# arkworks-rs/sponge

Measured on AMD Instinct MI355X. Metric: Poseidon permutations/sec (BLS12-381 Fr, t=3), higher is better.
Workload: dtype u32

## Files before the change

### sponge_amd/csrc/pmx_field.hpp

```cpp
#pragma once
#include <cstdint>
#include <type_traits>

#if defined(__HIPCC__)
#include <hip/hip_runtime.h>
#define PMX_FN __host__ __device__ __forceinline__
#else
#define PMX_FN inline
#endif

#if defined(PMX_HOSTCHECK) && !defined(__HIPCC__)
#define PMX_TRACK(tag, x, f) ::pmx::hostcheck_track(tag, x, f)
#else
#define PMX_TRACK(tag, x, f) ((void)0)
#endif

namespace pmx {

constexpr int kW = 29;
constexpr int kN = 9;
constexpr uint32_t kMask = (1u << kW) - 1;
constexpr int kFeStride = 12;

#if defined(__HIP_DEVICE_COMPILE__)
// ... 33 lines not shown
    uint32_t p[kN];
    uint32_t pinv;
    uint32_t unit;
    const uint32_t *io;
};
constexpr int kIoP32 = 0, kIoToInt = 8, kIoToAbi = 8 + kN, kIoFromU64 = 28, kIoWords = 40;

#if defined(PMX_HOSTCHECK) && !defined(__HIPCC__)
void hostcheck_track(int tag, const Fe &x, const FieldRt &f);
void hostcheck_below_2_256(const Fe &x);
#endif

PMX_FN Fe fe_const(const uint32_t *ptr) {
    Fe r;
#pragma unroll
    for (int i = 0; i < kN; ++i) r.l[i] = ptr[i];
    return r;
}

PMX_FN Fe fe_zero() {
    Fe z;
#pragma unroll
    for (int i = 0; i < kN; ++i) z.l[i] = 0;
    return z;
}

PMX_FN uint32_t mont_step(uint64_t &acc, const FieldRt &f) {
    const uint32_t m = ((uint32_t)acc * f.pinv) & kMask;
    acc += (uint64_t)m * f.p[0];
    acc >>= kW;
    return m;
}

PMX_FN Fe fe_add_lazy(const Fe &a, const Fe &b) {
    Fe r;
#pragma unroll
    for (int i = 0; i < kN; ++i) r.l[i] = a.l[i] + b.l[i];
    return r;
}

PMX_FN Fe fe_normalize(const Fe &a) {
    Fe r;
    uint32_t carry = 0;
#pragma unroll
    for (int i = 0; i < kN - 1; ++i) {
        const uint32_t v = a.l[i] + carry;
        r.l[i] = v & kMask;
        carry = v >> kW;
    }
    r.l[kN - 1] = a.l[kN - 1] + carry;
    return r;
}

template <int T, bool ADD>
PMX_FN Fe mont_dot_impl(const Fe *a, const Fe *b, const Fe &s, const FieldRt &f) {
    constexpr int G = (T + 2) / 3;
    uint32_t m[kN];
    Fe out;
    uint64_t acc[G];
#pragma unroll
    for (int g = 0; g < G; ++g) acc[g] = 0;
#pragma unroll
    for (int k = 0; k < 2 * kN - 1; ++k) {
        const int lo_i = k < kN ? 0 : k - (kN - 1);
        const int hi_i = k < kN ? k : kN - 1;
#pragma unroll
        for (int t = 0; t < T; ++t) {
#pragma unroll
            for (int i = lo_i; i <= hi_i; ++i) acc[t / 3] += (uint64_t)a[t].l[i] * b[t].l[k - i];
        }
#pragma unroll
        for (int j = lo_i; j <= hi_i; ++j) {
            if (j < k || k >= kN) acc[0] += (uint64_t)m[j] * f.p[k - j];
        }
        if constexpr (G == 1) {
            if (k < kN) {
                m[k] = mont_step(acc[0], f);
            } else {
                if constexpr (ADD) acc[0] += (uint64_t)s.l[k - kN] * f.unit;
                out.l[k - kN] = (uint32_t)acc[0] & kMask;
                acc[0] >>= kW;
            }
        } else {
            uint32_t low = (uint32_t)acc[0] & kMask;
            if constexpr (ADD) {
                if (k >= kN) low += s.l[k - kN];
            }
            uint64_t carry = acc[0] >> kW;
#pragma unroll
            for (int g = 1; g < G; ++g) {
                low += (uint32_t)acc[g] & kMask;
                carry += acc[g] >> kW;
                acc[g] = 0;
            }
            if (k < kN) {
                m[k] = (low * f.pinv) & kMask;
                const uint64_t v = (uint64_t)m[k] * f.p[0] + low;
                acc[0] = carry + (v >> kW);
            } else {
                out.l[k - kN] = low & kMask;
                acc[0] = carry + (low >> kW);
            }
        }
    }
    out.l[kN - 1] = (uint32_t)acc[0];
    if constexpr (ADD) out.l[kN - 1] += s.l[kN - 1];
    return out;
}

template <int T>
PMX_FN Fe mont_dot(const Fe *a, const Fe *b, const FieldRt &f) { return mont_dot_impl<T, false>(a, b, a[0], f); }
template <int T>
PMX_FN Fe mont_dot_add(const Fe *a, const Fe *b, const Fe &s, const FieldRt &f) { return mont_dot_impl<T, true>(a, b, s, f); }

PMX_FN Fe mont_mul(const Fe &a, const Fe &b, const FieldRt &f) { return mont_dot<1>(&a, &b, f); }

PMX_FN Fe mont_mul_add(const Fe &a, const Fe &b, const Fe &s, const FieldRt &f) {
    uint32_t m[kN];
    Fe out;
    uint64_t acc = 0;
#pragma unroll
    for (int k = 0; k < 2 * kN - 1; ++k) {
        const int lo_i = k < kN ? 0 : k - (kN - 1);
        const int hi_i = k < kN ? k : kN - 1;
#pragma unroll
        for (int i = lo_i; i <= hi_i; ++i) acc += (uint64_t)a.l[i] * b.l[k - i];
#pragma unroll
        for (int j = lo_i; j <= hi_i; ++j) {
            if (j < k || k >= kN) acc += (uint64_t)m[j] * f.p[k - j];
        }
        if (k < kN) {
            m[k] = mont_step(acc, f);
        } else {
            acc += (uint64_t)s.l[k - kN] * f.unit;
            out.l[k - kN] = (uint32_t)acc & kMask;
            acc >>= kW;
        }
    }
    out.l[kN - 1] = (uint32_t)acc + s.l[kN - 1];
    return out;
}

PMX_FN Fe mont_sqr(const Fe &a, const FieldRt &f) {
    uint32_t d[kN];
#pragma unroll
    for (int i = 0; i < kN; ++i) d[i] = a.l[i] << 1;
    uint32_t m[kN];
    Fe out;
    uint64_t acc = 0;
#pragma unroll
    for (int k = 0; k < 2 * kN - 1; ++k) {
#pragma unroll
        for (int i = 0; i < kN; ++i) {
            const int j = k - i;
            if (j > i && j < kN) acc += (uint64_t)a.l[i] * d[j];
        }
        if ((k & 1) == 0) acc += (uint64_t)a.l[k / 2] * a.l[k / 2];
        if (k < kN) {
#pragma unroll
            for (int j = 0; j < k; ++j) acc += (uint64_t)m[j] * f.p[k - j];
            m[k] = mont_step(acc, f);
        } else {
#pragma unroll
            for (int j = k - (kN - 1); j < kN; ++j) acc += (uint64_t)m[j] * f.p[k - j];
            out.l[k - kN] = (uint32_t)acc & kMask;
            acc >>= kW;
        }
    }
    out.l[kN - 1] = (uint32_t)acc;
    return out;
}

enum { kP1In = 0, kP1Sq = 1, kP1Out = 2 };
PMX_FN constexpr bool field_unit_low_limb(const uint32_t (&p)[kN]) { return p[0] == 1u; }

PMX_FN uint32_t mont_step_p1(uint64_t &acc) {
    const uint32_t n = ~(uint32_t)acc & kMask;
    acc >>= kW;
    return n;
}

PMX_FN Fe mont_mul_p1(const Fe &a, const Fe &b, const FieldRt &f) {
    uint32_t m[kN];
    Fe out;
    uint64_t acc = 0;
#pragma unroll
    for (int k = 0; k < 2 * kN - 1; ++k) {
        const int lo_i = k < kN ? 0 : k - (kN - 1);
        const int hi_i = k < kN ? k : kN - 1;
#pragma unroll
        for (int i = lo_i; i <= hi_i; ++i) acc += (uint64_t)a.l[i] * b.l[k - i];
#pragma unroll
        for (int j = lo_i; j <= hi_i; ++j) {
            if (j < k || k >= kN) acc += (uint64_t)m[j] * f.p[k - j];
        }
        if (k < kN) {
            if (k == kN - 1) acc += (uint64_t)1 << kW;
            m[k] = mont_step_p1(acc);
            if (k == 0) m[0] += 1;
        } else {
            out.l[k - kN] = (uint32_t)acc & kMask;
            acc >>= kW;
        }
    }
    out.l[kN - 1] = (uint32_t)acc;
    return out;
}

template <int MODE>
PMX_FN Fe mont_sqr_p1(const Fe &a, const FieldRt &f) {
    uint32_t d[kN];
#pragma unroll
    for (int i = 0; i < kN; ++i) d[i] = a.l[i] << 1;
    uint32_t m[kN];
    Fe out;
    uint64_t acc = MODE == kP1Sq ? ~(uint64_t)0 : (uint64_t)0;
#pragma unroll
    for (int k = 0; k < 2 * kN - 1; ++k) {
#pragma unroll
        for (int i = 0; i < kN; ++i) {
            const int j = k - i;
            if (j > i && j < kN) acc += (uint64_t)a.l[i] * d[j];
        }
        if ((k & 1) == 0) acc += (uint64_t)a.l[k / 2] * a.l[k / 2];
        if (k < kN) {
#pragma unroll
            for (int j = 0; j < k; ++j) acc += (uint64_t)m[j] * f.p[k - j];
            if (MODE == kP1Out && k == kN - 1) acc += (uint64_t)1 << kW;
            m[k] = mont_step_p1(acc);
            if (MODE != kP1Sq && k == 0) m[0] += 1;
        } else {
#pragma unroll
            for (int j = k - (kN - 1); j < kN; ++j) acc += (uint64_t)m[j] * f.p[k - j];
            out.l[k - kN] = (uint32_t)acc & kMask;
            acc >>= kW;
        }
    }
    out.l[kN - 1] = (uint32_t)acc;
    if (MODE != kP1Out) out.l[0] += 1;
    return out;
}

constexpr int kTabSteps = 2;
constexpr int kTabChunk = 3;
constexpr int kTabChunkWords = 32;
constexpr int kTabOneWords = (kN / kTabChunk) * kTabChunkWords;
PMX_FN constexpr int tab_row_words(int n) { return n == 1 ? kTabOneWords : kN * ((n + kTabChunk - 1) / kTabChunk) * kTabChunkWords; }
template <int N>
PMX_FN constexpr int tab_index(int i, int k, int j) {
    return N == 1 ? (k / kTabChunk) * kTabChunkWords + (k % kTabChunk) * kN + j
                  : (k * ((N + kTabChunk - 1) / kTabChunk) + i / kTabChunk) * kTabChunkWords + (i % kTabChunk) * kN + j;
}

PMX_FN void tab_col_end(int k, uint64_t &acc, uint32_t (&m)[kTabSteps], Fe &out, const Fe &s, const FieldRt &f) {
#pragma unroll
    for (int q = 0; q < kTabSteps; ++q) {
        if (q < k && k - q < kN) acc += (uint64_t)m[q] * f.p[k - q];
    }
    if (k < kTabSteps) {
// ... 38 lines not shown
            s[l] = out;
            acc = 0;
        }
        PMX_STREAM_FENCE(acc);
    });
}

struct Cols {
    uint64_t c[2 * kN];
};

PMX_FN void cols_zero(Cols &t) {
#pragma unroll
    for (int k = 0; k < 2 * kN; ++k) t.c[k] = 0;
}

PMX_FN void cols_mul_acc(Cols &t, const Fe &a, const Fe &b) {
#pragma unroll
    for (int i = 0; i < kN; ++i) {
#pragma unroll
        for (int j = 0; j < kN; ++j) t.c[i + j] += (uint64_t)a.l[i] * b.l[j];
    }
}

PMX_FN void cols_compress(Cols &t) {
#pragma unroll
    for (int k = 0; k < 2 * kN - 1; ++k) {
        t.c[k + 1] += t.c[k] >> kW;
        t.c[k] &= kMask;
    }
}

template <bool ADD = false>
PMX_FN Fe cols_redc(Cols &t, const FieldRt &f, const Fe *s = nullptr) {
#pragma unroll
    for (int k = 0; k < kN; ++k) {
        const uint32_t m = ((uint32_t)t.c[k] * f.pinv) & kMask;
#pragma unroll
        for (int j = 0; j < kN; ++j) t.c[k + j] += (uint64_t)m * f.p[j];
        t.c[k + 1] += t.c[k] >> kW;
    }
    Fe out;
#pragma unroll
    for (int k = kN; k < 2 * kN - 1; ++k) {
        if constexpr (ADD) t.c[k] += (uint64_t)s->l[k - kN] * f.unit;
        out.l[k - kN] = (uint32_t)t.c[k] & kMask;
        t.c[k + 1] += t.c[k] >> kW;
    }
    out.l[kN - 1] = (uint32_t)t.c[2 * kN - 1];
    if constexpr (ADD) out.l[kN - 1] += s->l[kN - 1];
    return out;
}

template <int ALPHA, bool P1 = false>
PMX_FN Fe fe_sbox(const Fe &x, uint64_t alpha, const Fe &one, const FieldRt &f) {
    if constexpr (P1 && ALPHA == 5) {
        const Fe x2 = mont_sqr_p1<kP1In>(x, f);
        const Fe x4 = mont_sqr_p1<kP1Sq>(x2, f);
        return mont_mul_p1(x4, x, f);
    } else if constexpr (P1 && ALPHA == 17) {
        Fe y = mont_sqr_p1<kP1In>(x, f);
        y = mont_sqr_p1<kP1Sq>(y, f);
        y = mont_sqr_p1<kP1Sq>(y, f);
        y = mont_sqr_p1<kP1Sq>(y, f);
        return mont_mul_p1(y, x, f);
    } else if constexpr (P1) {
        if (alpha == 0) return one;
        if (alpha == 1) return mont_mul_p1(x, one, f);
        const int top = 63 - __builtin_clzll(alpha);
        Fe acc = mont_sqr_p1<kP1Out>(x, f);
        if ((alpha >> (top - 1)) & 1) acc = mont_mul_p1(acc, x, f);
        for (int bit = top - 2; bit >= 0; --bit) {
            acc = mont_sqr_p1<kP1Out>(acc, f);
            if ((alpha >> bit) & 1) acc = mont_mul_p1(acc, x, f);
        }
        return acc;
    } else if constexpr (ALPHA == 5) {
        const Fe x2 = mont_sqr(x, f);
        const Fe x4 = mont_sqr(x2, f);
        return mont_mul(x4, x, f);
    } else if constexpr (ALPHA == 17) {
        Fe y = mont_sqr(x, f);
        y = mont_sqr(y, f);
        y = mont_sqr(y, f);
        y = mont_sqr(y, f);
        return mont_mul(y, x, f);
    } else {
        if (alpha == 0) return one;
        if (alpha == 1) return mont_mul(x, one, f);
        const int top = 63 - __builtin_clzll(alpha);
        Fe acc = mont_sqr(x, f);
        if ((alpha >> (top - 1)) & 1) acc = mont_mul(acc, x, f);
        for (int bit = top - 2; bit >= 0; --bit) {
            acc = mont_sqr(acc, f);
            if ((alpha >> bit) & 1) acc = mont_mul(acc, x, f);
        }
        return acc;
    }
}

PMX_FN Fe limbs_32_to_29(const Abi &x) {
    Fe r;
#pragma unroll
    for (int i = 0; i < kN; ++i) {
        const int bit = kW * i, wi = bit / 32, sh = bit % 32;
        uint64_t pair = x.w[wi];
        if (wi + 1 < 8) pair |= (uint64_t)x.w[wi + 1] << 32;
        r.l[i] = (uint32_t)(pair >> sh) & kMask;
    }
    return r;
}

PMX_FN Abi limbs_29_to_32(const Fe &x) {
    Abi r;
#pragma unroll
    for (int k = 0; k < 8; ++k) {
        const int bit = 32 * k, li = bit / kW, sh = bit % kW;
        uint64_t v = (uint64_t)x.l[li] >> sh;
        if (li + 1 < kN) v |= (uint64_t)x.l[li + 1] << (kW - sh);
        if (li + 2 < kN && 2 * kW - sh < 32) v |= (uint64_t)x.l[li + 2] << (2 * kW - sh);
        r.w[k] = (uint32_t)v;
    }
    return r;
}

PMX_FN Fe fe_from_abi(const Abi &x, const FieldRt &f) { return mont_mul(limbs_32_to_29(x), fe_const(f.io + kIoToInt), f); }

PMX_FN Abi fe_to_abi(const Fe &x, const FieldRt &f) {
    const Abi t = limbs_29_to_32(mont_mul(x, fe_const(f.io + kIoToAbi), f));
    uint32_t d[8];
    uint32_t borrow = 0;
#pragma unroll
    for (int i = 0; i < 8; ++i) {
        const uint64_t v = (uint64_t)t.w[i] - f.io[kIoP32 + i] - borrow;
        d[i] = (uint32_t)v;
        borrow = (uint32_t)(v >> 32) & 1u;
    }
    Abi r;
#pragma unroll
// ... 126 lines not shown
```

### sponge_amd/csrc/pmx_mfma.hpp

```cpp
#pragma once

#include "pmx_field.hpp"

namespace pmx {

#define PMX_MFMA_MIN_T 3
#define PMX_MFMA_MAX_T 9
constexpr int kMfmaElemBytes = 32;
constexpr int kMfmaShift = 24;
PMX_FN constexpr int mfma_k_steps(int t) { return (t * kMfmaElemBytes + 31) / 32; }
PMX_FN constexpr int mfma_row_words(int t) { return mfma_k_steps(t) * 64 * 4; }
PMX_FN constexpr int mfma_layer_words(int t) { return t * mfma_row_words(t) + t * 16; }
PMX_FN constexpr int mfma_layer_words_io(int n_in, int n_out) { return n_out * mfma_row_words(n_in) + n_out * 16; }

#ifndef PMX_MFMA_WINDOW
#define PMX_MFMA_WINDOW 9
#endif
PMX_FN constexpr int mfma_window_for(int t) {
    return (t >= PMX_MFMA_MIN_T && t <= PMX_MFMA_MAX_T) ? (PMX_MFMA_WINDOW < t ? PMX_MFMA_WINDOW : t) : 0;
}
PMX_FN constexpr int mfma_window_hist(int k) { return (k - 1) * (k - 2) / 2; }
constexpr int kMfmaMaxInputs = PMX_MFMA_MAX_T - 1 + (PMX_MFMA_WINDOW < PMX_MFMA_MAX_T ? PMX_MFMA_WINDOW : PMX_MFMA_MAX_T);
static_assert(32 * kMfmaMaxInputs * 128 * 128 < (1 << 25), "a sum of byte products must stay inside the accumulator budget of mfma_row_acc");
static_assert((unsigned long long)kMfmaMaxInputs * 32 * 255 < (1ull << kMfmaShift), "a row must stay below 2^256: n_in * 32 * 255 * p / 2^24 + p < 2 p");
PMX_FN constexpr bool mfma_row_pairs(int n_in) { return 257ll * 32 * n_in * (128 * 128) < (1ll << 31); }
static_assert(mfma_row_pairs(15), "pairs of byte sums fit 32 bits up to 15 inputs");
static_assert(!mfma_row_pairs(16), "... and no further: a row of 16 inputs or more keeps the four-weight finish");
static_assert(mfma_row_pairs(PMX_MFMA_MAX_T) && mfma_row_pairs(PMX_MFMA_MAX_T - 1), "dense layers and history rows (at most MAX_T - 1 inputs) take the paired finish");
#ifndef PMX_MFMA_HIST_TAB_MAX_T
#define PMX_MFMA_HIST_TAB_MAX_T 3
#endif
PMX_FN constexpr bool mfma_hist_tab(int t) { return t <= PMX_MFMA_HIST_TAB_MAX_T; }
constexpr uint32_t kMfmaHistSmallMarker = 0xffffffffu;
PMX_FN constexpr bool mfma_hist_rows(int t) { return !mfma_hist_tab(t); }
PMX_FN constexpr int mfma_fe_rows(int t) { return mfma_hist_rows(t) ? 2 : t; }
PMX_FN constexpr int mfma_hist_row_words(int k) { return mfma_k_steps(k) * 64 * 4 + 16; }
PMX_FN constexpr int mfma_hist_rows_offset(int k) {
    int w = 0;
    for (int j = 2; j < k; ++j) w += mfma_hist_row_words(j);
    return w;
}
PMX_FN constexpr int mfma_hist_row_input(int t, int k, int q) { return q < k - 1 ? t - 1 + q : k - 1; }
PMX_FN constexpr int mfma_hist_tab_offset(int k) {
    int w = 0;
    for (int j = 2; j < k; ++j) w += tab_row_words(j - 1);
    return w;
}
PMX_FN constexpr int mfma_window_hist_words(int t, int k) { return mfma_hist_tab(t) ? mfma_hist_tab_offset(k) : mfma_hist_rows_offset(k); }
PMX_FN constexpr size_t mfma_window_words(int t, int k, size_t windows) {
    return (size_t)mfma_layer_words(t) + windows * ((size_t)mfma_layer_words_io(t - 1 + k, t) + (size_t)mfma_window_hist_words(t, k));
}

PMX_FN void mfma_cut_element(const Fe &x, uint32_t *w8) {
#if defined(PMX_HOSTCHECK) && !defined(__HIPCC__)
    hostcheck_below_2_256(x);
#endif
#pragma unroll
    for (int w = 0; w < 8; ++w) {
        const int bit = 32 * w, li = bit / kW, sh = bit % kW;
        uint64_t v = (uint64_t)x.l[li] >> sh;
        if (li + 1 < kN) v |= (uint64_t)x.l[li + 1] << (kW - sh);
        if (li + 2 < kN && 2 * kW - sh < 32) v |= (uint64_t)x.l[li + 2] << (2 * kW - sh);
        w8[w] = (uint32_t)v ^ 0x80808080u;
    }
}
template <int T>
PMX_FN void mfma_state_words(const Fe *s, uint32_t (&W)[8 * mfma_k_steps(T)]) {
    static_assert(kMfmaElemBytes == 32 && mfma_k_steps(T) == T, "one k-step per element");
    static_for<0, T>([&](auto jj) { mfma_cut_element(s[decltype(jj)::value], &W[8 * decltype(jj)::value]); });
}

PMX_FN void mfma_row_acc_p(const int32_t (&R)[8][4], const long long *corr, const uint32_t *p32, uint32_t pinv, uint32_t (&a)[9]);
PMX_FN void mfma_row_acc(const int32_t (&R)[8][4], const long long *corr, const FieldRt &f, uint32_t (&a)[9]) {
    mfma_row_acc_p(R, corr, f.io + kIoP32, f.pinv, a);
}
PMX_FN void mfma_row_acc_p(const int32_t (&R)[8][4], const long long *corr, const uint32_t *p32, uint32_t pinv, uint32_t (&a)[9]) {
    int w1, w8, w16, w24;
#if defined(__HIP_DEVICE_COMPILE__)
    asm("v_mov_b32 %0, 1" : "=v"(w1));
    asm("v_mov_b32 %0, 0x100" : "=v"(w8));
    asm("v_mov_b32 %0, 0x10000" : "=v"(w16));
    asm("v_mov_b32 %0, 0x1000000" : "=v"(w24));
#else
    w1 = 1, w8 = 1 << 8, w16 = 1 << 16, w24 = 1 << 24;
#endif
    int carry = 0;
    uint32_t m = 0;
#pragma unroll
    for (int w = 0; w < 8; ++w) {
        long long t = corr[w] + (long long)carry * w1;
        t += (long long)R[w][0] * w1;
        t += (long long)R[w][1] * w8;
        t += (long long)R[w][2] * w16;
        t += (long long)R[w][3] * w24;
        if (w == 0) m = ((uint32_t)t * pinv) & 0xffffffu;
        t = (long long)((uint64_t)m * p32[w] + (uint64_t)t);
        a[w] = (uint32_t)t;
        carry = (int)(t >> 32);
    }
    a[8] = (uint32_t)carry;
}
#if defined(PMX_HOSTCHECK) && !defined(__HIPCC__)
void hostcheck_pair_fits_32(long long q) __attribute__((weak));
#endif
PMX_FN int32_t mfma_pair_sums(int32_t lo, int32_t hi) {
#if defined(PMX_HOSTCHECK) && !defined(__HIPCC__)
    if (hostcheck_pair_fits_32) hostcheck_pair_fits_32((long long)lo + 256ll * (long long)hi);
#endif
    return (int32_t)(((uint32_t)hi << 8) + (uint32_t)lo);
}
PMX_FN void mfma_row_acc_pairs_p(const int32_t (&Q)[8][2], const long long *corr, const uint32_t *p32, uint32_t pinv, uint32_t (&a)[9]) {
    int w1, w16;
#if defined(__HIP_DEVICE_COMPILE__)
    asm("v_mov_b32 %0, 1" : "=v"(w1));
    asm("v_mov_b32 %0, 0x10000" : "=v"(w16));
#else
    w1 = 1, w16 = 1 << 16;
#endif
    int carry = 0;
    uint32_t m = 0;
#pragma unroll
    for (int w = 0; w < 8; ++w) {
        long long t = corr[w] + (long long)carry * w1;
        t += (long long)Q[w][0] * w1;
        t += (long long)Q[w][1] * w16;
        if (w == 0) m = ((uint32_t)t * pinv) & 0xffffffu;
        t = (long long)((uint64_t)m * p32[w] + (uint64_t)t);
        a[w] = (uint32_t)t;
        carry = (int)(t >> 32);
    }
    a[8] = (uint32_t)carry;
}
template <int NIN>
PMX_FN void mfma_row_acc_for(const int32_t (&R)[8][4], const long long *corr, const uint32_t *p32, uint32_t pinv, uint32_t (&a)[9]) {
    if constexpr (mfma_row_pairs(NIN)) {
        int32_t Q[8][2];
#pragma unroll
        for (int w = 0; w < 8; ++w) Q[w][0] = mfma_pair_sums(R[w][0], R[w][1]), Q[w][1] = mfma_pair_sums(R[w][2], R[w][3]);
        mfma_row_acc_pairs_p(Q, corr, p32, pinv, a);
    } else {
        mfma_row_acc_p(R, corr, p32, pinv, a);
    }
}
PMX_FN uint32_t mfma_row_bits(const uint32_t (&a)[9], int bit) {
    const int wi = bit / 32, sh = bit % 32;
    const uint32_t lo = a[wi], hi = wi + 1 < 9 ? a[wi + 1] : 0u;
#if defined(__HIP_DEVICE_COMPILE__)
    return sh == 0 ? lo : __builtin_amdgcn_alignbit(hi, lo, sh);
#else
    return (uint32_t)((((uint64_t)hi << 32) | lo) >> sh);
#endif
}
PMX_FN Fe mfma_row_limbs(const uint32_t (&a)[9]) {
    Fe row;
#pragma unroll
    for (int k = 0; k < kN; ++k) {
        const uint32_t v = mfma_row_bits(a, kMfmaShift + kW * k);
        row.l[k] = k + 1 < kN ? (v & kMask) : v;
    }
    return row;
}
PMX_FN Fe mfma_row_finish(const int32_t (&R)[8][4], const long long *corr, const FieldRt &f) {
    uint32_t a[9];
    mfma_row_acc(R, corr, f, a);
    return mfma_row_limbs(a);
}

#if defined(__HIPCC__)
__device__ __forceinline__ void lane32_swap(uint32_t &x, uint32_t &y);
#endif
PMX_FN Fe mfma_row_operand(const uint32_t (&a)[9]);
PMX_FN Fe mfma_row_finish_operand(const int32_t (&R)[8][4], const long long *corr, const FieldRt &f) {
    uint32_t a[9];
    mfma_row_acc(R, corr, f, a);
    return mfma_row_operand(a);
}
PMX_FN Fe mfma_row_operand(const uint32_t (&a)[9]) {
    Fe row;
#pragma unroll
    for (int k = 0; k < 8; ++k) row.l[k] = mfma_row_bits(a, kMfmaShift + 32 * k) ^ 0x80808080u;
    row.l[8] = 0;
#if defined(__HIP_DEVICE_COMPILE__)
#pragma unroll
    for (int u = 0; u < 4; ++u) lane32_swap(row.l[u], row.l[4 + u]);
#endif
    return row;
}
PMX_FN void mfma_copy_operand(const Fe &x, uint32_t *w8) {
#pragma unroll
    for (int w = 0; w < 8; ++w) w8[w] = x.l[w];
}

#if !defined(__HIPCC__)
template <int NQ>
inline Fe mfma_row_host(const uint32_t *W, const uint32_t *layer, size_t n_rows, uint32_t i, const FieldRt &f, bool as_element = true) {
    const int8_t *bytes = reinterpret_cast<const int8_t *>(layer);
    const long long *corr = reinterpret_cast<const long long *>(layer + n_rows * (size_t)(NQ * 64 * 4));
    int32_t R[8][4];
    for (int e = 0; e < 32; ++e) {
        long long sum = 0;
        for (int k = 0; k < 32 * NQ; ++k) {
            const int u = (int)(int8_t)((W[k / 4] >> (8 * (k % 4))) & 0xff);
            const int q = k / 32, h = (k % 32) / 16, byte = k % 16;
            sum += (long long)u * bytes[(((size_t)i * NQ + q) * 64 + 32 * h + e) * 16 + byte];
        }
        R[e / 4][e % 4] = (int32_t)sum;
    }
    uint32_t a[9];
    mfma_row_acc_for<NQ>(R, corr + (size_t)i * 8, f.io + kIoP32, f.pinv, a);
    return as_element ? mfma_row_limbs(a) : mfma_row_operand(a);
}
inline void mfma_cut_operand(const Fe &x, uint32_t *w8) { mfma_cut_element(x, w8); }
template <int NIN, int NOUT, class Scratch>
inline void matrix_rows_mfma_w(const uint32_t (&W)[8 * NIN], Fe *out, Scratch &sc, const uint32_t *layer, const FieldRt &f, uint32_t lo, uint32_t hi,
                               uint32_t fe_rows = NOUT) {
    Fe last = out[NOUT - 1];
    for (uint32_t i = lo; i < hi; ++i) {
        const Fe row = mfma_row_host<NIN>(W, layer, NOUT, i, f, i < fe_rows);
        if (i + 1 < (uint32_t)NOUT) sc.set(i, row);
        else last = row;
    }
    static_for<0, NOUT - 1>([&](auto i) { out[i] = sc.get(i); });
    out[NOUT - 1] = last;
}
template <int NIN, int NOUT, class Scratch>
inline void matrix_rows_mfma_io(const Fe *in, Fe *out, Scratch &sc, const uint32_t *layer, const FieldRt &f, uint32_t lo, uint32_t hi,
                                uint32_t fe_rows = NOUT) {
    uint32_t W[8 * NIN];
    mfma_state_words<NIN>(in, W);
    matrix_rows_mfma_w<NIN, NOUT>(W, out, sc, layer, f, lo, hi, fe_rows);
}
template <int T, class Scratch>
inline void matrix_rows_mfma(Fe (&s)[T], Scratch &sc, const uint32_t *layer, const FieldRt &f, uint32_t lo, uint32_t hi, uint32_t fe_rows = T) {
    matrix_rows_mfma_io<T, T>(s, s, sc, layer, f, lo, hi, fe_rows);
}
template <int T>
struct MfmaHistRow {
    const uint32_t *loaded = nullptr, *table = nullptr;
    uint32_t Wc[8 * PMX_MFMA_WINDOW];
    template <int KK>
    void load(const uint32_t *tab) { loaded = tab; }
    template <int KK, int NW>
    void products(const uint32_t (&W)[NW]) {
        table = loaded;
        static_for<0, KK>([&](auto qq) {
            constexpr int q = decltype(qq)::value, g = mfma_hist_row_input(T, KK, q);
            for (int w = 0; w < 8; ++w) Wc[8 * q + w] = W[8 * g + w];
        });
    }
    template <int KK>
    Fe finish(const FieldRt &f) { return mfma_row_host<KK>(Wc, table, 1, 0, f); }
};
#endif

#if defined(__HIPCC__)

typedef int mfma_v16i __attribute__((ext_vector_type(16)));
typedef int mfma_v4i __attribute__((ext_vector_type(4)));

__device__ __forceinline__ void lane32_swap(uint32_t &x, uint32_t &y) {
    const auto r = __builtin_amdgcn_permlane32_swap(x, y, false, false);
    x = r[0];
    y = r[1];
}

template <int NIN>
__device__ __forceinline__ void mfma_row_home(const mfma_v16i &d1, const mfma_v16i &d2, const long long *corr, const uint32_t *p32, uint32_t pinv,
                                              uint32_t (&a)[9]) {
    if constexpr (mfma_row_pairs(NIN)) {
        int32_t Q[8][2];
#pragma unroll
        for (int v = 0; v < 8; ++v) {
            const int g = v / 2, h = v % 2;
            uint32_t x = (uint32_t)mfma_pair_sums(d1[4 * g + 2 * h], d1[4 * g + 2 * h + 1]);
            uint32_t y = (uint32_t)mfma_pair_sums(d2[4 * g + 2 * h], d2[4 * g + 2 * h + 1]);
            lane32_swap(x, y);
            Q[2 * g][h] = (int32_t)x;
            Q[2 * g + 1][h] = (int32_t)y;
        }
        mfma_row_acc_pairs_p(Q, corr, p32, pinv, a);
    } else {
        int32_t R4[8][4];
#pragma unroll
        for (int v = 0; v < 16; ++v) {
            uint32_t x = (uint32_t)d1[v], y = (uint32_t)d2[v];
            lane32_swap(x, y);
            R4[2 * (v / 4)][v % 4] = (int32_t)x;
// ... 28 lines not shown
    const uint32_t lane_off = lane * 16u;
    auto kstep = [&](uint32_t row, int q) -> mfma_v4i {
        const uint32_t soff = (row * (uint32_t)NQ + (uint32_t)(q & ~3)) * 1024u;
        const auto v = __builtin_amdgcn_raw_buffer_load_b128(rsrc, lane_off + (uint32_t)(q & 3) * 1024u, soff, 0);
        return mfma_v4i{(int)v[0], (int)v[1], (int)v[2], (int)v[3]};
    };
    Fe last = out[T - 1];
    mfma_v4i a[SLOTS];
    if (lo < hi) {
#pragma unroll
        for (int q = 0; q < R; ++q) {
            a[q] = kstep(lo, q);
            PMX_SCHED_FENCE();
        }
#pragma unroll
        for (int e = 0; e < REM; ++e) {
            a[R + e] = kstep(lo, FULL + e);
            PMX_SCHED_FENCE();
        }
    }
#pragma clang loop unroll(disable) vectorize(disable) interleave(disable)
    for (uint32_t i = lo; i < hi; ++i) {
        const uint32_t nxt = i + 1 < hi ? i + 1 : i;
        mfma_v16i d1 = {0, 0, 0, 0, 0, 0, 0, 0, 0, 0, 0, 0, 0, 0, 0, 0}, d2 = d1;
        long long cw[8];
        uint32_t pw[8];
#pragma unroll
        for (int w = 0; w < 8; ++w) cw[w] = corr[(size_t)i * 8 + w], pw[w] = f.io[kIoP32 + w];
        PMX_SCHED_FENCE();
        static_for<0, NQ>([&](auto qq) {
            constexpr int q = decltype(qq)::value;
            constexpr int slot = q < FULL ? q % R : R + (q - FULL);
            const mfma_v4i b1 = {(int)W[8 * q + 0], (int)W[8 * q + 1], (int)W[8 * q + 2], (int)W[8 * q + 3]};
            const mfma_v4i b2 = {(int)W[8 * q + 4], (int)W[8 * q + 5], (int)W[8 * q + 6], (int)W[8 * q + 7]};
            d1 = __builtin_amdgcn_mfma_i32_32x32x32_i8(a[slot], b1, d1, 0, 0, 0);
            d2 = __builtin_amdgcn_mfma_i32_32x32x32_i8(a[slot], b2, d2, 0, 0, 0);
            PMX_SCHED_FENCE();
            if constexpr (q + R < FULL) a[slot] = kstep(i, q + R);
            else if constexpr (q < FULL) a[slot] = kstep(nxt, q % R);
            else a[slot] = kstep(nxt, q);
            PMX_SCHED_FENCE();
        });
        Fe row;
        uint32_t acc9[9];
        mfma_row_home<NIN>(d1, d2, cw, pw, f.pinv, acc9);
        if (!kOperandRows || i < fe_rows) row = mfma_row_limbs(acc9);
        else row = mfma_row_operand(acc9);
        if (i + 1 < (uint32_t)T) sc.set(i, row);
        else last = row;
    }
    static_for<0, T - 1>([&](auto i) { out[i] = sc.get(i); });
    out[T - 1] = last;
}
template <int NIN, int NOUT, class Scratch>
__device__ __forceinline__ void matrix_rows_mfma_io(const Fe *in, Fe *out, Scratch &sc, const uint32_t *layer, const FieldRt &f,
                                                    uint32_t lo, uint32_t hi, uint32_t fe_rows = NOUT) {
    uint32_t W[8 * NIN];
    static_for<0, NIN>([&](auto j) { mfma_cut_operand(in[decltype(j)::value], &W[8 * decltype(j)::value]); });
    matrix_rows_mfma_w<NIN, NOUT>(W, out, sc, layer, f, lo, hi, fe_rows);
}
template <int T, class Scratch>
__device__ __forceinline__ void matrix_rows_mfma(Fe (&s)[T], Scratch &sc, const uint32_t *layer, const FieldRt &f, uint32_t lo,
                                                 uint32_t hi, uint32_t fe_rows = T) {
    matrix_rows_mfma_io<T, T>(s, s, sc, layer, f, lo, hi, fe_rows);
}

template <int T>
struct MfmaHistRow {
    mfma_v4i a[PMX_MFMA_WINDOW > 2 ? PMX_MFMA_WINDOW - 1 : 1];
    mfma_v16i d1, d2;
    const long long *loaded_corr, *corr;
    template <int KK>
    __device__ __forceinline__ void load(const uint32_t *table) {
        const mfma_v4i *src = reinterpret_cast<const mfma_v4i *>(table) + (threadIdx.x & 63);
#pragma unroll
        for (int q = 0; q < KK; ++q) a[q] = src[q * 64];
        loaded_corr = reinterpret_cast<const long long *>(table + (size_t)mfma_k_steps(KK) * 64 * 4);
    }
    template <int KK, int NW>
    __device__ __forceinline__ void products(const uint32_t (&W)[NW]) {
        const mfma_v16i zero = {0, 0, 0, 0, 0, 0, 0, 0, 0, 0, 0, 0, 0, 0, 0, 0};
        d1 = zero, d2 = zero;
        corr = loaded_corr;
        static_for<0, KK>([&](auto qq) {
            constexpr int q = decltype(qq)::value, g = mfma_hist_row_input(T, KK, q);
            const mfma_v4i b1 = {(int)W[8 * g + 0], (int)W[8 * g + 1], (int)W[8 * g + 2], (int)W[8 * g + 3]};
            const mfma_v4i b2 = {(int)W[8 * g + 4], (int)W[8 * g + 5], (int)W[8 * g + 6], (int)W[8 * g + 7]};
            d1 = __builtin_amdgcn_mfma_i32_32x32x32_i8(a[q], b1, d1, 0, 0, 0);
            d2 = __builtin_amdgcn_mfma_i32_32x32x32_i8(a[q], b2, d2, 0, 0, 0);
        });
    }
    template <int KK>
    __device__ __forceinline__ Fe finish(const FieldRt &f) {
        uint32_t acc9[9];
        mfma_row_home<KK>(d1, d2, corr, f.io + kIoP32, f.pinv, acc9);
        return mfma_row_limbs(acc9);
    }
};

#endif

}
```

### sponge_amd/csrc/pmx_permute.hpp

```cpp
#pragma once
#include "pmx_field.hpp"
#include "pmx_mfma.hpp"

namespace pmx {

struct Rounds {
    uint32_t rate, capacity, half_full, partial_rounds, total_rounds;
    uint64_t alpha;
};

PMX_FN bool is_full_round(uint32_t r, const Rounds &c) {
    return r < c.half_full || r >= c.half_full + c.partial_rounds;
}

struct OptTables {
    const uint32_t *ark;
    const uint32_t *mfma;
    const uint32_t *win;
};

PMX_FN uint32_t full_ordinal(uint32_t r, const Rounds &c) { return r < c.half_full ? r : r - c.partial_rounds - 1; }

template <int T, int ALPHA, class Scratch, int MFMA_WINDOW, bool P1 = false>
PMX_FN void permute_hybrid(Fe (&s)[T], Scratch &sc, const OptTables &tb, const Rounds &c, const Fe &one,
                           const FieldRt &f, uint32_t want_lo = 0, uint32_t want_hi = T, bool lane0_zero = false) {
    static_assert(MFMA_WINDOW > 0 && MFMA_WINDOW <= T, "a window is at most as long as the state is wide");
    const uint32_t first_partial = c.half_full, last_partial = c.half_full + c.partial_rounds - 1;
    for (uint32_t r = 0; r < c.total_rounds; ++r) {
        if (r == first_partial) {
            constexpr int K = MFMA_WINDOW, NIN = T - 1 + K;
            constexpr size_t kLayer = (size_t)mfma_layer_words_io(NIN, T), kPer = kLayer + (size_t)mfma_window_hist_words(T, K);
            const uint32_t n_win = (c.partial_rounds + K - 1) / K;
            uint32_t kw = c.partial_rounds - (n_win - 1) * K;
            const uint32_t *wt = tb.win + mfma_layer_words(T);
#pragma clang loop unroll(disable) vectorize(disable) interleave(disable)
            for (uint32_t w = 0; w < n_win; ++w, wt += kPer, kw = K) {
                const uint32_t *hist = wt + kLayer;
                if constexpr (mfma_hist_rows(T)) {
                    uint32_t W[8 * NIN];
                    static_for<1, T>([&](auto i) {
                        if constexpr ((int)i < mfma_fe_rows(T)) mfma_cut_operand(s[i], &W[8 * (i - 1)]);
                        else mfma_copy_operand(s[i], &W[8 * (i - 1)]);
                    });
                    MfmaHistRow<T> hr;
                    constexpr bool kFetchAhead = T != 5 && T != 9;
                    if constexpr (K > 2 && kFetchAhead) hr.template load<2>(hist);
                    Fe z = fe_sbox<ALPHA, P1>(s[0], c.alpha, one, f);
                    mfma_cut_operand(z, &W[8 * (T - 1)]);
                    Fe x = fe_add_lazy(s[1], z);
                    static_for<2, K + 1>([&](auto kk) {
                        constexpr int k = decltype(kk)::value;
                        if ((uint32_t)k <= kw) {
                            const bool row = k < K && (uint32_t)k < kw;
                            z = fe_sbox<ALPHA, P1>(x, c.alpha, one, f);
                            mfma_cut_operand(z, &W[8 * (T - 2 + k)]);
                            if constexpr (k < K) {
                                if (row) {
                                    if constexpr (!kFetchAhead) hr.template load<k>(hist + mfma_hist_rows_offset(k));
                                    hr.template products<k>(W);
                                    if constexpr (k + 1 < K && kFetchAhead) hr.template load<k + 1>(hist + mfma_hist_rows_offset(k + 1));
                                    x = fe_add_lazy(hr.template finish<k>(f), z);
                                }
                            }
                        } else {
                            mfma_cut_operand(fe_zero(), &W[8 * (T - 2 + k)]);
                        }
                    });
                    const uint32_t fe_rows = w + 1 < n_win ? (uint32_t)mfma_fe_rows(T) : (uint32_t)T;
                    matrix_rows_mfma_w<NIN, T>(W, s, sc, wt, f, 0u, (uint32_t)T, fe_rows);
                } else {
                    static_assert(K <= 3, "the table form of the history terms covers the single term of a window of three");
                    Fe in[NIN];
                    static_for<1, T>([&](auto i) { in[i - 1] = s[i]; });
                    in[T - 1] = fe_sbox<ALPHA, P1>(s[0], c.alpha, one, f);
                    static_for<1, K>([&](auto kk) {
                        constexpr int k = decltype(kk)::value;
                        if ((uint32_t)k < kw) {
                            Fe x = s[k];
                            bool small_sum = false;
                            if constexpr (k == 2) {
                                const uint32_t small = hist[0] == kMfmaHistSmallMarker ? hist[1] : 0u;
                                if (small) {
                                    small_sum = true;
                                    x = fe_add_lazy(x, in[T - 1]);
                                    if (small >= 2) x = fe_add_lazy(x, in[T - 1]);
                                    if (small >= 3) x = fe_add_lazy(x, in[T - 1]);
                                    if (small >= 4) x = fe_add_lazy(x, in[T - 1]);
                                } else {
                                    PMX_SCHED_FENCE();
                                    tab_lanes_stream<1>(in[T - 1], hist, &x, f);
                                    PMX_SCHED_FENCE();
                                }
                            }
                            x = fe_add_lazy(x, in[T - 2 + k]);
                            if (small_sum) x = fe_normalize(x);
                            in[T - 1 + k] = fe_sbox<ALPHA, P1>(x, c.alpha, one, f);
                        } else {
                            in[T - 1 + k] = fe_zero();
                        }
                    });
                    matrix_rows_mfma_io<NIN, T>(in, s, sc, wt, f, 0u, (uint32_t)T);
                }
            }
            r = last_partial;
            continue;
        }
        const uint32_t *rk = tb.ark + (size_t)r * T * kFeStride;
        static_for<0, T - 1>([&](auto i) { sc.set(i, s[i]); });
        uint32_t first = 0;
        if (r == 0 && lane0_zero && c.half_full > 0) {
            const uint32_t n_win = (c.partial_rounds + MFMA_WINDOW - 1) / MFMA_WINDOW;
            sc.set(0, fe_const(tb.win + mfma_window_words(T, MFMA_WINDOW, n_win)));
            first = 1;
        }
#pragma clang loop unroll(disable) vectorize(disable) interleave(disable)
        for (uint32_t i = first; i + 1 < (uint32_t)T; ++i)
            sc.set(i, fe_sbox<ALPHA, P1>(fe_add_lazy(sc.get(i), fe_const(rk + i * kFeStride)), c.alpha, one, f));
        s[T - 1] = fe_sbox<ALPHA, P1>(fe_add_lazy(s[T - 1], fe_const(rk + (T - 1) * kFeStride)), c.alpha, one, f);
        static_for<0, T - 1>([&](auto i) { s[i] = sc.get(i); });
        const bool last = r + 1 == c.total_rounds, entrance = r + 1 == first_partial;
        const uint32_t *lay = tb.mfma + (size_t)full_ordinal(r, c) * mfma_layer_words(T);
        uint32_t fe_rows = (uint32_t)T;
        if (entrance) {
            lay = tb.win;
            fe_rows = (uint32_t)mfma_fe_rows(T);
        }
        matrix_rows_mfma<T>(s, sc, lay, f, last ? want_lo : 0u, last ? want_hi : (uint32_t)T, fe_rows);
    }
}

constexpr int kCoopElems = 4;

template <int ALPHA>
PMX_FN Fe coop_pre(const Fe &s, const uint32_t *entry, bool apply_sbox, const Rounds &c, const Fe &one, const FieldRt &f) {
    const Fe x = fe_add_lazy(s, fe_const(entry));
    const Fe y = fe_sbox<ALPHA>(x, c.alpha, one, f);
    Fe z;
#pragma unroll
    for (int w = 0; w < kN; ++w) z.l[w] = apply_sbox ? y.l[w] : x.l[w];
    return z;
}

PMX_FN Fe coop_post(const Fe (&z)[3], const uint32_t *entry, const FieldRt &f) {
    Fe row[3];
    static_for<0, 3>([&](auto j) { row[j] = fe_const(entry + (1 + j) * kFeStride); });
    return mont_dot<3>(z, row, f);
}
PMX_FN Fe coop_post_norm(const Fe (&z)[3], const uint32_t *entry, const FieldRt &f) {
    Fe row[3];
    static_for<1, 3>([&](auto j) { row[j] = fe_const(entry + (1 + j) * kFeStride); });
    return mont_dot_add<2>(&z[1], &row[1], z[0], f);
}
PMX_FN bool coop_layer_is_norm(uint32_t r, const Rounds &c) {
    const uint32_t last_partial = c.half_full + c.partial_rounds - 1;
    return r == last_partial || (is_full_round(r, c) && r + 1 != c.half_full && r + 1 != c.total_rounds);
}

template <int ALPHA>
constexpr bool kCoopFolded = ALPHA == 5 || ALPHA == 17;
template <int ALPHA>
constexpr int kCoopExtraSquarings = ALPHA == 17 ? 2 : 0;

PMX_FN Fe fe_select(bool c, const Fe &a, const Fe &b) {
    Fe r;
#pragma unroll
    for (int w = 0; w < kN; ++w) r.l[w] = c ? a.l[w] : b.l[w];
    return r;
}

PMX_FN Fe coop_fold_a(uint32_t q, const Fe &x, const uint32_t *entry, const FieldRt &f) {
    return mont_mul(x, fe_select(q == 3, x, fe_const(entry + kFeStride)), f);
}
PMX_FN Fe coop_fold_b(uint32_t q, const Fe &s, const Fe &res_a, const uint32_t *entry, const FieldRt &f) {
    return mont_mul(fe_select(q == 3, res_a, s), fe_select(q == 3, res_a, fe_const(entry + 2 * kFeStride)), f);
}
PMX_FN Fe coop_fold_c(uint32_t q, const Fe &s, const Fe &xpow, const Fe &res_a, const Fe &p1, const Fe &p2, const FieldRt &f) {
    return mont_mul_add(xpow, res_a, fe_select(q == 0, fe_add_lazy(p1, p2), s), f);
}

constexpr uint32_t kRtLazyTerms = 3;
// ... 34 lines not shown
```

Baseline: 892.3 million.

## Emit MFMA operand words directly from the S-box's final Montgomery multiply

```diff
diff --git a/sponge_amd/csrc/pmx_field.hpp b/sponge_amd/csrc/pmx_field.hpp
--- a/sponge_amd/csrc/pmx_field.hpp
+++ b/sponge_amd/csrc/pmx_field.hpp
@@ -109,8 +109,28 @@
     return r;
 }
 
-template <int T, bool ADD>
-PMX_FN Fe mont_dot_impl(const Fe *a, const Fe *b, const Fe &s, const FieldRt &f) {
+enum { kOutLimbs = 1, kOutWords = 2, kOutBoth = 3 };
+constexpr uint32_t kOperandBias = 0x80808080u;
+template <int FORM>
+PMX_FN void fe_out_column(int j, uint32_t lo, Fe &out, Fe &words) {
+    if constexpr ((FORM & kOutLimbs) != 0) out.l[j] = j + 1 < kN ? (lo & kMask) : lo;
+    if constexpr ((FORM & kOutWords) != 0) {
+        if (j > 0) words.l[j - 1] = (words.l[j - 1] | (lo << (32 - 3 * j))) ^ kOperandBias;
+        if (j + 1 < kN) words.l[j] = (lo >> (3 * j)) & ((1u << (kW - 3 * j)) - 1u);
+        else words.l[j] = 0;
+    }
+}
+#if defined(PMX_HOSTCHECK) && !defined(__HIPCC__)
+#define PMX_OUT_FORM(FORM) ((FORM) | kOutLimbs)
+#define PMX_OUT_CHECK(FORM, out) do { if (((FORM) & kOutWords) != 0) ::pmx::hostcheck_below_2_256(out); } while (0)
+#else
+#define PMX_OUT_FORM(FORM) (FORM)
+#define PMX_OUT_CHECK(FORM, out) ((void)0)
+#endif
+
+template <int T, bool ADD, int FORM = kOutLimbs>
+PMX_FN Fe mont_dot_impl(const Fe *a, const Fe *b, const Fe &s, const FieldRt &f, Fe &words) {
+    static_assert(FORM == kOutLimbs || (T == 1 && !ADD), "only a single product has an operand-word form");
     constexpr int G = (T + 2) / 3;
     uint32_t m[kN];
     Fe out;
@@ -135,7 +155,7 @@
                 m[k] = mont_step(acc[0], f);
             } else {
                 if constexpr (ADD) acc[0] += (uint64_t)s.l[k - kN] * f.unit;
-                out.l[k - kN] = (uint32_t)acc[0] & kMask;
+                fe_out_column<PMX_OUT_FORM(FORM)>(k - kN, (uint32_t)acc[0], out, words);
                 acc[0] >>= kW;
             }
         } else {
@@ -160,17 +180,30 @@
             }
         }
     }
-    out.l[kN - 1] = (uint32_t)acc[0];
+    if constexpr (G == 1) {
+        fe_out_column<PMX_OUT_FORM(FORM)>(kN - 1, (uint32_t)acc[0], out, words);
+    } else {
+        out.l[kN - 1] = (uint32_t)acc[0];
+    }
     if constexpr (ADD) out.l[kN - 1] += s.l[kN - 1];
+    PMX_OUT_CHECK(FORM, out);
     return out;
 }
 
 template <int T>
-PMX_FN Fe mont_dot(const Fe *a, const Fe *b, const FieldRt &f) { return mont_dot_impl<T, false>(a, b, a[0], f); }
+PMX_FN Fe mont_dot(const Fe *a, const Fe *b, const FieldRt &f) {
+    Fe none;
+    return mont_dot_impl<T, false>(a, b, a[0], f, none);
+}
 template <int T>
-PMX_FN Fe mont_dot_add(const Fe *a, const Fe *b, const Fe &s, const FieldRt &f) { return mont_dot_impl<T, true>(a, b, s, f); }
+PMX_FN Fe mont_dot_add(const Fe *a, const Fe *b, const Fe &s, const FieldRt &f) {
+    Fe none;
+    return mont_dot_impl<T, true>(a, b, s, f, none);
+}
 
 PMX_FN Fe mont_mul(const Fe &a, const Fe &b, const FieldRt &f) { return mont_dot<1>(&a, &b, f); }
+template <int FORM>
+PMX_FN Fe mont_mul(const Fe &a, const Fe &b, const FieldRt &f, Fe &words) { return mont_dot_impl<1, false, FORM>(&a, &b, a, f, words); }
 
 PMX_FN Fe mont_mul_add(const Fe &a, const Fe &b, const Fe &s, const FieldRt &f) {
     uint32_t m[kN];
@@ -237,7 +270,8 @@
     return n;
 }
 
-PMX_FN Fe mont_mul_p1(const Fe &a, const Fe &b, const FieldRt &f) {
+template <int FORM>
+PMX_FN Fe mont_mul_p1(const Fe &a, const Fe &b, const FieldRt &f, Fe &words) {
     uint32_t m[kN];
     Fe out;
     uint64_t acc = 0;
@@ -256,12 +290,17 @@
             m[k] = mont_step_p1(acc);
             if (k == 0) m[0] += 1;
         } else {
-            out.l[k - kN] = (uint32_t)acc & kMask;
+            fe_out_column<PMX_OUT_FORM(FORM)>(k - kN, (uint32_t)acc, out, words);
             acc >>= kW;
         }
     }
-    out.l[kN - 1] = (uint32_t)acc;
+    fe_out_column<PMX_OUT_FORM(FORM)>(kN - 1, (uint32_t)acc, out, words);
+    PMX_OUT_CHECK(FORM, out);
     return out;
+}
+PMX_FN Fe mont_mul_p1(const Fe &a, const Fe &b, const FieldRt &f) {
+    Fe none;
+    return mont_mul_p1<kOutLimbs>(a, b, f, none);
 }
 
 template <int MODE>
@@ -406,18 +445,45 @@
     return out;
 }
 
+PMX_FN void mfma_cut_element(const Fe &x, uint32_t *w8);
 template <int ALPHA, bool P1 = false>
-PMX_FN Fe fe_sbox(const Fe &x, uint64_t alpha, const Fe &one, const FieldRt &f) {
+PMX_FN Fe fe_sbox(const Fe &x, uint64_t alpha, const Fe &one, const FieldRt &f);
+template <int ALPHA, bool P1, int FORM>
+PMX_FN Fe fe_sbox(const Fe &x, uint64_t alpha, const Fe &one, const FieldRt &f, Fe &words) {
     if constexpr (P1 && ALPHA == 5) {
         const Fe x2 = mont_sqr_p1<kP1In>(x, f);
         const Fe x4 = mont_sqr_p1<kP1Sq>(x2, f);
-        return mont_mul_p1(x4, x, f);
+        return mont_mul_p1<FORM>(x4, x, f, words);
     } else if constexpr (P1 && ALPHA == 17) {
         Fe y = mont_sqr_p1<kP1In>(x, f);
         y = mont_sqr_p1<kP1Sq>(y, f);
         y = mont_sqr_p1<kP1Sq>(y, f);
         y = mont_sqr_p1<kP1Sq>(y, f);
-        return mont_mul_p1(y, x, f);
+        return mont_mul_p1<FORM>(y, x, f, words);
+    } else if constexpr (ALPHA == 5) {
+        const Fe x2 = mont_sqr(x, f);
+        const Fe x4 = mont_sqr(x2, f);
+        return mont_mul<FORM>(x4, x, f, words);
+    } else if constexpr (ALPHA == 17) {
+        Fe y = mont_sqr(x, f);
+        y = mont_sqr(y, f);
+        y = mont_sqr(y, f);
+        y = mont_sqr(y, f);
+        return mont_mul<FORM>(y, x, f, words);
+    } else {
+        const Fe z = fe_sbox<ALPHA, P1>(x, alpha, one, f);
+        if constexpr ((FORM & kOutWords) != 0) {
+            mfma_cut_element(z, words.l);
+            words.l[kN - 1] = 0;
+        }
+        return z;
+    }
+}
+template <int ALPHA, bool P1>
+PMX_FN Fe fe_sbox(const Fe &x, uint64_t alpha, const Fe &one, const FieldRt &f) {
+    if constexpr (ALPHA == 5 || ALPHA == 17) {
+        Fe none;
+        return fe_sbox<ALPHA, P1, kOutLimbs>(x, alpha, one, f, none);
     } else if constexpr (P1) {
         if (alpha == 0) return one;
         if (alpha == 1) return mont_mul_p1(x, one, f);
@@ -429,16 +495,6 @@
             if ((alpha >> bit) & 1) acc = mont_mul_p1(acc, x, f);
         }
         return acc;
-    } else if constexpr (ALPHA == 5) {
-        const Fe x2 = mont_sqr(x, f);
-        const Fe x4 = mont_sqr(x2, f);
-        return mont_mul(x4, x, f);
-    } else if constexpr (ALPHA == 17) {
-        Fe y = mont_sqr(x, f);
-        y = mont_sqr(y, f);
-        y = mont_sqr(y, f);
-        y = mont_sqr(y, f);
-        return mont_mul(y, x, f);
     } else {
         if (alpha == 0) return one;
         if (alpha == 1) return mont_mul(x, one, f);
diff --git a/sponge_amd/csrc/pmx_mfma.hpp b/sponge_amd/csrc/pmx_mfma.hpp
--- a/sponge_amd/csrc/pmx_mfma.hpp
+++ b/sponge_amd/csrc/pmx_mfma.hpp
@@ -64,11 +64,6 @@
         w8[w] = (uint32_t)v ^ 0x80808080u;
     }
 }
-template <int T>
-PMX_FN void mfma_state_words(const Fe *s, uint32_t (&W)[8 * mfma_k_steps(T)]) {
-    static_assert(kMfmaElemBytes == 32 && mfma_k_steps(T) == T, "one k-step per element");
-    static_for<0, T>([&](auto jj) { mfma_cut_element(s[decltype(jj)::value], &W[8 * decltype(jj)::value]); });
-}
 
 PMX_FN void mfma_row_acc_p(const int32_t (&R)[8][4], const long long *corr, const uint32_t *p32, uint32_t pinv, uint32_t (&a)[9]);
 PMX_FN void mfma_row_acc(const int32_t (&R)[8][4], const long long *corr, const FieldRt &f, uint32_t (&a)[9]) {
@@ -175,15 +170,20 @@
     mfma_row_acc(R, corr, f, a);
     return mfma_row_operand(a);
 }
+PMX_FN void mfma_words_to_operand(Fe &words) {
+#if defined(__HIP_DEVICE_COMPILE__)
+#pragma unroll
+    for (int u = 0; u < 4; ++u) lane32_swap(words.l[u], words.l[4 + u]);
+#else
+    (void)words;
+#endif
+}
 PMX_FN Fe mfma_row_operand(const uint32_t (&a)[9]) {
     Fe row;
 #pragma unroll
-    for (int k = 0; k < 8; ++k) row.l[k] = mfma_row_bits(a, kMfmaShift + 32 * k) ^ 0x80808080u;
+    for (int k = 0; k < 8; ++k) row.l[k] = mfma_row_bits(a, kMfmaShift + 32 * k) ^ kOperandBias;
     row.l[8] = 0;
-#if defined(__HIP_DEVICE_COMPILE__)
-#pragma unroll
-    for (int u = 0; u < 4; ++u) lane32_swap(row.l[u], row.l[4 + u]);
-#endif
+    mfma_words_to_operand(row);
     return row;
 }
 PMX_FN void mfma_copy_operand(const Fe &x, uint32_t *w8) {
@@ -222,17 +222,6 @@
     }
     static_for<0, NOUT - 1>([&](auto i) { out[i] = sc.get(i); });
     out[NOUT - 1] = last;
-}
-template <int NIN, int NOUT, class Scratch>
-inline void matrix_rows_mfma_io(const Fe *in, Fe *out, Scratch &sc, const uint32_t *layer, const FieldRt &f, uint32_t lo, uint32_t hi,
-                                uint32_t fe_rows = NOUT) {
-    uint32_t W[8 * NIN];
-    mfma_state_words<NIN>(in, W);
-    matrix_rows_mfma_w<NIN, NOUT>(W, out, sc, layer, f, lo, hi, fe_rows);
-}
-template <int T, class Scratch>
-inline void matrix_rows_mfma(Fe (&s)[T], Scratch &sc, const uint32_t *layer, const FieldRt &f, uint32_t lo, uint32_t hi, uint32_t fe_rows = T) {
-    matrix_rows_mfma_io<T, T>(s, s, sc, layer, f, lo, hi, fe_rows);
 }
 template <int T>
 struct MfmaHistRow {
@@ -367,18 +356,6 @@
     static_for<0, T - 1>([&](auto i) { out[i] = sc.get(i); });
     out[T - 1] = last;
 }
-template <int NIN, int NOUT, class Scratch>
-__device__ __forceinline__ void matrix_rows_mfma_io(const Fe *in, Fe *out, Scratch &sc, const uint32_t *layer, const FieldRt &f,
-                                                    uint32_t lo, uint32_t hi, uint32_t fe_rows = NOUT) {
-    uint32_t W[8 * NIN];
-    static_for<0, NIN>([&](auto j) { mfma_cut_operand(in[decltype(j)::value], &W[8 * decltype(j)::value]); });
-    matrix_rows_mfma_w<NIN, NOUT>(W, out, sc, layer, f, lo, hi, fe_rows);
-}
-template <int T, class Scratch>
-__device__ __forceinline__ void matrix_rows_mfma(Fe (&s)[T], Scratch &sc, const uint32_t *layer, const FieldRt &f, uint32_t lo,
-                                                 uint32_t hi, uint32_t fe_rows = T) {
-    matrix_rows_mfma_io<T, T>(s, s, sc, layer, f, lo, hi, fe_rows);
-}
 
 template <int T>
 struct MfmaHistRow {
diff --git a/sponge_amd/csrc/pmx_permute.hpp b/sponge_amd/csrc/pmx_permute.hpp
--- a/sponge_amd/csrc/pmx_permute.hpp
+++ b/sponge_amd/csrc/pmx_permute.hpp
@@ -21,10 +21,32 @@
 
 PMX_FN uint32_t full_ordinal(uint32_t r, const Rounds &c) { return r < c.half_full ? r : r - c.partial_rounds - 1; }
 
+template <int ALPHA, bool P1, int FORM>
+PMX_FN Fe sbox_operand(const Fe &x, const Rounds &c, const Fe &one, const FieldRt &f, Fe &words) {
+    const Fe z = fe_sbox<ALPHA, P1, FORM>(x, c.alpha, one, f, words);
+    mfma_words_to_operand(words);
+    return z;
+}
+template <int ALPHA, bool P1, int FORM, bool WORDS = true>
+PMX_FN Fe sbox_operand(const Fe &x, const Rounds &c, const Fe &one, const FieldRt &f, uint32_t *w8) {
+    if constexpr (WORDS) {
+        Fe words;
+        const Fe z = sbox_operand<ALPHA, P1, FORM>(x, c, one, f, words);
+        mfma_copy_operand(words, w8);
+        return z;
+    } else {
+        const Fe z = fe_sbox<ALPHA, P1>(x, c.alpha, one, f);
+        mfma_cut_operand(z, w8);
+        return z;
+    }
+}
+PMX_FN constexpr bool sbox_words_for(int t) { return t <= 8; }
+
 template <int T, int ALPHA, class Scratch, int MFMA_WINDOW, bool P1 = false>
 PMX_FN void permute_hybrid(Fe (&s)[T], Scratch &sc, const OptTables &tb, const Rounds &c, const Fe &one,
                            const FieldRt &f, uint32_t want_lo = 0, uint32_t want_hi = T, bool lane0_zero = false) {
     static_assert(MFMA_WINDOW > 0 && MFMA_WINDOW <= T, "a window is at most as long as the state is wide");
+    constexpr bool kWords = sbox_words_for(T);
     const uint32_t first_partial = c.half_full, last_partial = c.half_full + c.partial_rounds - 1;
     for (uint32_t r = 0; r < c.total_rounds; ++r) {
         if (r == first_partial) {
@@ -45,15 +67,13 @@
                     MfmaHistRow<T> hr;
                     constexpr bool kFetchAhead = T != 5 && T != 9;
                     if constexpr (K > 2 && kFetchAhead) hr.template load<2>(hist);
-                    Fe z = fe_sbox<ALPHA, P1>(s[0], c.alpha, one, f);
-                    mfma_cut_operand(z, &W[8 * (T - 1)]);
+                    Fe z = sbox_operand<ALPHA, P1, kOutBoth, kWords>(s[0], c, one, f, &W[8 * (T - 1)]);
                     Fe x = fe_add_lazy(s[1], z);
                     static_for<2, K + 1>([&](auto kk) {
                         constexpr int k = decltype(kk)::value;
                         if ((uint32_t)k <= kw) {
                             const bool row = k < K && (uint32_t)k < kw;
-                            z = fe_sbox<ALPHA, P1>(x, c.alpha, one, f);
-                            mfma_cut_operand(z, &W[8 * (T - 2 + k)]);
+                            z = sbox_operand<ALPHA, P1, (k < K ? kOutBoth : kOutWords), kWords>(x, c, one, f, &W[8 * (T - 2 + k)]);
                             if constexpr (k < K) {
                                 if (row) {
                                     if constexpr (!kFetchAhead) hr.template load<k>(hist + mfma_hist_rows_offset(k));
@@ -70,9 +90,9 @@
                     matrix_rows_mfma_w<NIN, T>(W, s, sc, wt, f, 0u, (uint32_t)T, fe_rows);
                 } else {
                     static_assert(K <= 3, "the table form of the history terms covers the single term of a window of three");
-                    Fe in[NIN];
-                    static_for<1, T>([&](auto i) { in[i - 1] = s[i]; });
-                    in[T - 1] = fe_sbox<ALPHA, P1>(s[0], c.alpha, one, f);
+                    uint32_t W[8 * NIN];
+                    Fe zl[K];
+                    zl[0] = sbox_operand<ALPHA, P1, (K > 1 ? kOutBoth : kOutWords)>(s[0], c, one, f, &W[8 * (T - 1)]);
                     static_for<1, K>([&](auto kk) {
                         constexpr int k = decltype(kk)::value;
                         if ((uint32_t)k < kw) {
@@ -82,24 +102,25 @@
                                 const uint32_t small = hist[0] == kMfmaHistSmallMarker ? hist[1] : 0u;
                                 if (small) {
                                     small_sum = true;
-                                    x = fe_add_lazy(x, in[T - 1]);
-                                    if (small >= 2) x = fe_add_lazy(x, in[T - 1]);
-                                    if (small >= 3) x = fe_add_lazy(x, in[T - 1]);
-                                    if (small >= 4) x = fe_add_lazy(x, in[T - 1]);
+                                    x = fe_add_lazy(x, zl[0]);
+                                    if (small >= 2) x = fe_add_lazy(x, zl[0]);
+                                    if (small >= 3) x = fe_add_lazy(x, zl[0]);
+                                    if (small >= 4) x = fe_add_lazy(x, zl[0]);
                                 } else {
                                     PMX_SCHED_FENCE();
-                                    tab_lanes_stream<1>(in[T - 1], hist, &x, f);
+                                    tab_lanes_stream<1>(zl[0], hist, &x, f);
                                     PMX_SCHED_FENCE();
                                 }
                             }
-                            x = fe_add_lazy(x, in[T - 2 + k]);
+                            x = fe_add_lazy(x, zl[k - 1]);
                             if (small_sum) x = fe_normalize(x);
-                            in[T - 1 + k] = fe_sbox<ALPHA, P1>(x, c.alpha, one, f);
+                            zl[k] = sbox_operand<ALPHA, P1, (k + 1 < K ? kOutBoth : kOutWords)>(x, c, one, f, &W[8 * (T - 1 + k)]);
                         } else {
-                            in[T - 1 + k] = fe_zero();
+                            mfma_cut_operand(fe_zero(), &W[8 * (T - 1 + k)]);
                         }
                     });
-                    matrix_rows_mfma_io<NIN, T>(in, s, sc, wt, f, 0u, (uint32_t)T);
+                    static_for<1, T>([&](auto i) { mfma_cut_operand(s[i], &W[8 * (i - 1)]); });
+                    matrix_rows_mfma_w<NIN, T>(W, s, sc, wt, f, 0u, (uint32_t)T);
                 }
             }
             r = last_partial;
@@ -110,14 +131,33 @@
         uint32_t first = 0;
         if (r == 0 && lane0_zero && c.half_full > 0) {
             const uint32_t n_win = (c.partial_rounds + MFMA_WINDOW - 1) / MFMA_WINDOW;
-            sc.set(0, fe_const(tb.win + mfma_window_words(T, MFMA_WINDOW, n_win)));
+            Fe z0 = fe_const(tb.win + mfma_window_words(T, MFMA_WINDOW, n_win));
+            if constexpr (kWords) {
+                const Fe limbs = z0;
+                z0 = fe_zero();
+                mfma_cut_operand(limbs, z0.l);
+            }
+            sc.set(0, z0);
             first = 1;
         }
-#pragma clang loop unroll(disable) vectorize(disable) interleave(disable)
-        for (uint32_t i = first; i + 1 < (uint32_t)T; ++i)
-            sc.set(i, fe_sbox<ALPHA, P1>(fe_add_lazy(sc.get(i), fe_const(rk + i * kFeStride)), c.alpha, one, f));
-        s[T - 1] = fe_sbox<ALPHA, P1>(fe_add_lazy(s[T - 1], fe_const(rk + (T - 1) * kFeStride)), c.alpha, one, f);
-        static_for<0, T - 1>([&](auto i) { s[i] = sc.get(i); });
+        uint32_t W[8 * T];
+        if constexpr (kWords) {
+#pragma clang loop unroll(disable) vectorize(disable) interleave(disable)
+            for (uint32_t i = first; i + 1 < (uint32_t)T; ++i) {
+                Fe zw;
+                sbox_operand<ALPHA, P1, kOutWords>(fe_add_lazy(sc.get(i), fe_const(rk + i * kFeStride)), c, one, f, zw);
+                sc.set(i, zw);
+            }
+            sbox_operand<ALPHA, P1, kOutWords>(fe_add_lazy(s[T - 1], fe_const(rk + (T - 1) * kFeStride)), c, one, f, &W[8 * (T - 1)]);
+            static_for<0, T - 1>([&](auto i) { mfma_copy_operand(sc.get(i), &W[8 * i]); });
+        } else {
+#pragma clang loop unroll(disable) vectorize(disable) interleave(disable)
+            for (uint32_t i = first; i + 1 < (uint32_t)T; ++i)
+                sc.set(i, fe_sbox<ALPHA, P1>(fe_add_lazy(sc.get(i), fe_const(rk + i * kFeStride)), c.alpha, one, f));
+            s[T - 1] = fe_sbox<ALPHA, P1>(fe_add_lazy(s[T - 1], fe_const(rk + (T - 1) * kFeStride)), c.alpha, one, f);
+            static_for<0, T - 1>([&](auto i) { mfma_cut_operand(sc.get(i), &W[8 * i]); });
+            mfma_cut_operand(s[T - 1], &W[8 * (T - 1)]);
+        }
         const bool last = r + 1 == c.total_rounds, entrance = r + 1 == first_partial;
         const uint32_t *lay = tb.mfma + (size_t)full_ordinal(r, c) * mfma_layer_words(T);
         uint32_t fe_rows = (uint32_t)T;
@@ -125,7 +165,7 @@
             lay = tb.win;
             fe_rows = (uint32_t)mfma_fe_rows(T);
         }
-        matrix_rows_mfma<T>(s, sc, lay, f, last ? want_lo : 0u, last ? want_hi : (uint32_t)T, fe_rows);
+        matrix_rows_mfma_w<T, T>(W, s, sc, lay, f, last ? want_lo : 0u, last ? want_hi : (uint32_t)T, fe_rows);
     }
 }
 
```

Result: no change. 897.7 million (median of 6 runs) (+0.6%).
